# ZhenlongYuan/TSAR-MVS

Hardware: AMD Instinct MI355X
Metric: depthmap Mpixels/sec (ETH3D full-res, 8 iters) (higher is better)
Workload: dtype f32

## Files before the change

### tsar-mvs_amd/csrc/pm_core.h

```cpp
#pragma once
#include <type_traits>

#include "tsar_device_math.h"

#define PM_BLOCK 256
#define PM_RW 32

#include "pm_tap_common.h"

template <bool QUAD, bool DIFF = false>
DEVFN float sample_bilinear(const DevView& vw, int w, int h, int qpitch, float u, float v, bool q8 = false) {
    u = fminf(fmaxf(u, -1.0f), (float)w);
    v = fminf(fmaxf(v, -1.0f), (float)h);
    const float fu = floorf(u), fv = floorf(v);
    float ax = u - fu, ay = v - fv;
    if (q8) { ax = rintf(ax * 256.0f) * 0.00390625f; ay = rintf(ay * 256.0f) * 0.00390625f; }
    const int iu = (int)fu, iv = (int)fv;
    float t00, t10, t01, t11;
    if (QUAD) {
        const uint32_t off = (uint32_t)(__mul24(iv + 1, qpitch) + iu + 1) * 4u;
        const uint32_t q = *(global_u32_ptr)((const char __attribute__((address_space(1)))*)vw.quad + off);
        t00 = (float)(q & 0xffu);
        t10 = (float)((q >> 8) & 0xffu);
        t01 = (float)((q >> 16) & 0xffu);
// ... 130 lines not shown
DEVFN float add_prior_term(const DevScene* __restrict__ sc, int x, int y, const float4& n4, float D, float c) {
    const float4* pp = sc->prior;
    if (pp == nullptr) return c;
    typedef float prior_entry __attribute__((ext_vector_type(4)));
    const prior_entry q = ((const __attribute__((address_space(1))) prior_entry*)pp)[y * sc->w + x];
    const float Dp = q.w;
    const float a = fabsf(D - Dp);
    const float rel = a / Dp;
    const float dclip = sc->prior_depth_clip, nclip = sc->prior_normal_clip;
    const float r_d = rel < dclip ? rel / dclip : 1.0f;
    const float s = 1.0f - ((n4.x * q.x + n4.y * q.y) + n4.z * q.z);
    const float s0 = s < 0.0f ? 0.0f : s;
    const float r_n = s < nclip ? s0 / nclip : 1.0f;
    const float t = (sc->prior_weight_depth * r_d) + (sc->prior_weight_normal * r_n);
    return Dp > 0.0f ? c + t : c;
}

template <int NB, int HR, bool STRICT, bool QUAD, int V = 0, int BLK = PM_BLOCK>
DEVFN float multiview_cost(const DevScene* __restrict__ sc, const typename TileOf<QUAD>::type* tile, int tw, int own, const float* wts, const PixelRef& pr,
                           int x, int y, const float4& n4, int& beview, float& ratio, bool prune = false, float cost_now = 0.0f, int* skipped = nullptr) {
    constexpr bool GEOM = (V & TSAR_V_GEOM) != 0;
    constexpr bool PRUNE = (V & TSAR_V_PRUNE) != 0;
    static_assert(!PRUNE || !GEOM, "the bound speaks of the photometric cost alone");
    constexpr int VT = V & ~(TSAR_V_GEOM | TSAR_V_REDRAW | TSAR_V_PRUNE);
    float best[NB];
#pragma unroll
    for (int k = 0; k < NB; k++) best[k] = __builtin_inff();
    const int num = sc->n_sel;
    int valid = 0, bv = -1;
    float cmin = __builtin_inff();
    float depth_h = 0.0f;
    if constexpr (GEOM) depth_h = plane_depth(sc->ref, n4, x, y);
    int vi_next = sc->sel[0];
    for (int i = 0; i < num; i++) {
        const int vi = vi_next;
        vi_next = sc->sel[i + 1 < num ? i + 1 : i];
        float c;
        if constexpr ((VT & TSAR_V_LUT) != 0) c = view_cost_lut<STRICT, (VT >> 11) & 7, (VT & TSAR_V_BUF) != 0 && !STRICT, (VT & TSAR_V_MIX) != 0 && !STRICT>(sc, sc->view[vi], tile, tw, own, wts, pr, x, y, n4);
        else if constexpr (QUAD && HR == 5 && r5_production_variant(VT) && PRUNE) {
            static_assert((VT & 250) == 250 && !STRICT, "pruning instantiations exist for the fast row-wise loop");
            ViewPrune vp;
            vp.on = prune; vp.skipped = false;
            vp.cost_now = cmin < cost_now ? TSAR_MAXCOST : cost_now;
            c = view_cost_r5<false, true, true, (VT & TSAR_V_BUF) != 0, (VT & TSAR_V_MIX) != 0, BLK, 0, true>(sc, sc->view[vi], tile, tw, own, wts, pr, x, y, n4, &vp);
            if (vp.skipped) *skipped += 1;
        } else if constexpr (QUAD && HR == 5 && r5_production_variant(VT))
            c = view_cost_r5<STRICT, (VT & 128) != 0 && !STRICT, (VT & 8) != 0, (VT & TSAR_V_BUF) != 0, (VT & TSAR_V_MIX) != 0, BLK>(sc, sc->view[vi], tile, tw, own, wts, pr, x, y, n4);
#ifdef TSAR_EXPERIMENTS
        else if constexpr (QUAD && HR == 5 && r5_diag_variant(VT))
            c = view_cost_r5<false, true, true, true, true, BLK, (VT & 4194304) ? 1 : 2>(sc, sc->view[vi], tile, tw, own, wts, pr, x, y, n4);
#endif
        else {
            static_assert(VT == 0, "unknown tap-loop variant");
            c = view_cost_generic<HR, STRICT, QUAD, BLK>(sc, sc->view[vi], tile, tw, own, wts, pr, x, y, n4);
        }
        auto vmin = [](float a, float b) { float r; asm("v_min_f32 %0, %1, %2" : "=v"(r) : "v"(a), "v"(b)); return r; };
        auto vmax = [](float a, float b) { float r; asm("v_max_f32 %0, %1, %2" : "=v"(r) : "v"(a), "v"(b)); return r; };
        c = vmin(c, TSAR_MAXCOST);
        valid -= (int32_t)__float_as_uint(c - TSAR_MAXCOST) >> 31;
        if constexpr (GEOM) c = c + geom_term(sc, sc->view[vi], vi, x, y, depth_h);
        {
            const uint32_t worse = (uint32_t)((int32_t)__float_as_uint(cmin - c) >> 31);
            asm("v_bfi_b32 %0, %1, %2, %3" : "=v"(bv) : "v"(worse), "v"(bv), "s"(vi));
            cmin = vmin(cmin, c);
        }
        float v = c;
#pragma unroll
        for (int k = 0; k < NB; k++) {
            const float lo = vmin(best[k], v), hi = vmax(best[k], v);
            best[k] = lo;
            v = hi;
// ... 37 lines not shown
```

### tsar-mvs_amd/csrc/pm_init.hip

```cpp
#include "pm_init_impl.h"

template <bool INIT, bool REDRAW = false>
static int launch_full(tsar_ctx* ctx, const float4* planes, float* c, float4* n, int32_t* bv, float* rt) {
    if (every_pixel_takes_lut(ctx)) return launch_pm_full_lut(ctx, INIT, REDRAW, planes, c, n, bv, rt);
    return with_tap_config(ctx, [&](auto cfg) { return launch_full_g<decltype(cfg), INIT, REDRAW>(cfg, ctx, planes, c, n, bv, rt); });
}

int launch_pm_init(tsar_ctx* ctx) { return launch_full<true>(ctx, nullptr, ctx->buf[0].c, ctx->buf[0].n4, nullptr, nullptr); }
int launch_pm_cost_planes(tsar_ctx* ctx, const float4* planes, float* cost, int32_t* beview, float* ratio) {
    return launch_full<false>(ctx, planes, cost, nullptr, beview, ratio);
}
int launch_pm_rescore(tsar_ctx* ctx, const float4* planes, float* cost, float4* n, int32_t* beview, float* ratio) {
    return launch_full<true, true>(ctx, planes, cost, n, beview, ratio);
}
```

### tsar-mvs_amd/csrc/pm_init_impl.h

```cpp
#pragma once
#include "pm_dispatch.h"

#define FULL_RH 8

template <int NB, int HR, bool STRICT, bool QUAD, bool INIT, int V = 0>
__global__ __launch_bounds__(PM_BLOCK) void pm_full_kernel(const DevScene* __restrict__ sc, const float4* __restrict__ planes_in,
                                                           float* __restrict__ c_out, float4* __restrict__ n_out,
                                                           int32_t* __restrict__ beview_out, float* __restrict__ ratio_out, int tiles_x,
                                                           int n_tiles, int strip_w) {
    extern __shared__ __attribute__((aligned(16))) unsigned char lds_raw[];
    typedef typename TileOf<QUAD>::type TileT;
    const int hr = HR > 0 ? HR : sc->hrad, vr = HR > 0 ? HR : sc->vrad;
    const int tw = PM_RW + 2 * hr, th = FULL_RH + 2 * vr;
    constexpr bool LUTW = (V & TSAR_V_LUT) != 0;
    const size_t lut_bytes = LUTW ? (size_t)(sc->lut_classes + 1) * 1024 : 0;
    TileT* tile = (TileT*)(lds_raw + lut_bytes);
    float* wts = LUTW ? (float*)lds_raw : (float*)(lds_raw + tile_bytes<QUAD>(tw, th)) + threadIdx.x;
    if constexpr (LUTW) build_weight_lut<PM_BLOCK>(sc, wts);
    const int t = xcd_tile(blockIdx.x, n_tiles);
    int tix, tiy;
    strip_tile(t, tiles_x, n_tiles / tiles_x, strip_w, tix, tiy);
    const int ty0 = tiy * FULL_RH, tx0 = tix * PM_RW;
    stage_ref_tile<FULL_RH, TileT>(sc, tile, tx0, ty0, hr, vr, LUTW ? LUT_TILE_PAD_ROWS : 0);
    __syncthreads();
// ... 41 lines not shown
        n4 = planes_in[p];
    }
    if constexpr (REDRAW) n_out[p] = n4;
    PixelRef pr;
    if constexpr (LUTW) pr = hoist_reference_lut(sc, tile, tw, own, wts);
    else pr = hoist_reference<HR, TileT>(tile, tw, own, wts, hr, vr);
    float cost = TSAR_MAXCOST, rt = 0.f;
    int bv = -1;
    if (pr.textured) cost = multiview_cost<NB, HR, STRICT, QUAD, V>(sc, tile, tw, own, wts, pr, x, y, n4, bv, rt);
    c_out[p] = cost;
    if (!INIT || REDRAW) {
        if (beview_out) beview_out[p] = bv;
        if (ratio_out) ratio_out[p] = rt;
    }
}

template <int NB, int HR, bool STRICT, bool QUAD, bool INIT, int V = 0>
static int launch_full_t(tsar_ctx* ctx, const float4* planes, float* c, float4* n, int32_t* bv, float* rt) {
    auto kern = pm_full_kernel<NB, HR, STRICT, QUAD, INIT, V>;
    TapGrid g;
    if (const int rc = tap_grid(ctx, kern, FULL_RH, PM_BLOCK, QUAD, V, 0, g)) return rc;
    {
        ScopedKernelTimer tm(ctx, (INIT && (V & TSAR_V_REDRAW)) ? "pm_rescore" : INIT ? "pm_init" : "pm_cost_planes");
        hipLaunchKernelGGL(kern, dim3(g.n_tiles), dim3(PM_BLOCK), g.lds, ctx->stream, ctx->dscene, planes, c, n, bv, rt, g.tiles_x, g.n_tiles, strip_width(ctx->strip_w, g.tiles_x));
    }
    TSAR_HIP_TRY(ctx, hipGetLastError());
    return TSAR_OK;
}

template <class Cfg, bool INIT, bool REDRAW = false>
static int launch_full_g(Cfg, tsar_ctx* ctx, const float4* planes, float* c, float4* n, int32_t* bv, float* rt) {
    constexpr int NB = Cfg::NB, HR = Cfg::HR, V = Cfg::V;
    constexpr bool STRICT = Cfg::STRICT, QUAD = Cfg::QUAD;
    static_assert(INIT || !REDRAW, "only the initialising form redraws");
    if constexpr (REDRAW) return launch_full_t<NB, HR, STRICT, QUAD, true, V | TSAR_V_GEOM | TSAR_V_REDRAW>(ctx, planes, c, n, bv, rt);
    else if (scene_has_terms(ctx->hscene)) return launch_full_t<NB, HR, STRICT, QUAD, INIT, V | TSAR_V_GEOM>(ctx, planes, c, n, bv, rt);
    else return launch_full_t<NB, HR, STRICT, QUAD, INIT, V>(ctx, planes, c, n, bv, rt);
}
```

### tsar-mvs_amd/csrc/pm_sweep.hip

```cpp
#include "pm_sweep_impl.h"

__global__ void d16_probe_kernel(uint32_t* out) {
    __shared__ unsigned short t[64];
    t[threadIdx.x] = (unsigned short)(0x4300u + threadIdx.x);
    __syncthreads();
    uint32_t r = 0xffffffffu;
    const uint32_t addr = (uint32_t)(uintptr_t)(const __attribute__((address_space(3))) unsigned short*)(t + threadIdx.x);
    asm volatile("ds_read_u16_d16_hi %0, %1\n\ts_waitcnt lgkmcnt(0)" : "+v"(r) : "v"(addr));
    out[threadIdx.x] = r;
}
bool probe_d16_hi_zeroes(tsar_ctx* ctx) {
    CallFrame f(ctx, "d16 probe", nullptr, false);
    uint32_t h[64];
    uint32_t* d = f.out(h, 64, TSAR_MEM_HOST);
    if (f.ok()) {
        hipLaunchKernelGGL(d16_probe_kernel, dim3(1), dim3(64), 0, ctx->stream, d);
        f.launched();
    }
    bool ok = f.finish() == TSAR_OK;
    for (int i = 0; ok && i < 64; i++) ok = h[i] == ((0x4300u + i) << 16);
    return ok;
}

template <int NB, int HR>
static int launch_sweep_nh(tsar_ctx* ctx, int colour, const PlaneBuf& a, const PlaneBuf& b, const PlaneBuf& c, uint32_t sid, int dp, int dr) {
    const bool strict = ctx->hscene.flags & TSAR_FLAG_STRICT_DIV, quad = ctx->hscene.use_quad;
    const bool buf = ctx->buffer_gather && ctx->sweeps_done >= (strict ? (ctx->buffer_from > 2 ? ctx->buffer_from : 2) : ctx->buffer_from);
    const int v = ctx->variant;
    if constexpr ((NB == 2 || NB == 4) && HR == 5)
    if (quad && !(ctx->hscene.flags & TSAR_FLAG_TEX_FILTER_8BIT) && (v == 250 || v == 122 || (v == 114 && NB == 2))) {
#define SWEEP_R5(S, V, B) (buf ? launch_sweep_g<NB, 5, S, true, (V) | TSAR_V_BUF, B>(ctx, colour, a, b, c, sid, dp, dr) : launch_sweep_g<NB, 5, S, true, V, B>(ctx, colour, a, b, c, sid, dp, dr))
        const bool mix = buf && !strict && v == 250 && ctx->hscene.n_sel > 0 && ctx->hscene.view[ctx->hscene.sel[0]].dquad != nullptr;
#define SWEEP_R5_FAST250_ALL(B) (mix ? launch_sweep_g<NB, 5, false, true, 250 | TSAR_V_BUF | TSAR_V_MIX, B>(ctx, colour, a, b, c, sid, dp, dr) : SWEEP_R5(false, 250, B))
        const bool prune = NB == 2 && !strict && v == 250 && ctx->prune && ctx->prune_steps > 0 && dr && ctx->call_launch >= ctx->prune_from &&
                           ctx->hscene.cost_comb == TSAR_COMB_BEST_N && ctx->hscene.n_best == 1 && !scene_has_terms(ctx->hscene);
#define SWEEP_R5_PRUNE(B) (mix ? launch_sweep_t<2, 5, false, true, 250 | TSAR_V_BUF | TSAR_V_MIX | TSAR_V_PRUNE, B>(ctx, colour, a, b, c, sid, dp, dr) \
                           : buf ? launch_sweep_t<2, 5, false, true, 250 | TSAR_V_BUF | TSAR_V_PRUNE, B>(ctx, colour, a, b, c, sid, dp, dr)              \
                                 : launch_sweep_t<2, 5, false, true, 250 | TSAR_V_PRUNE, B>(ctx, colour, a, b, c, sid, dp, dr))
#define SWEEP_R5_FAST250(B) (prune ? SWEEP_R5_PRUNE(B) : SWEEP_R5_FAST250_ALL(B))
        if constexpr (NB == 2) {
            const int tiles256 = ((ctx->hscene.w + PM_RW - 1) / PM_RW) * ((ctx->hscene.h + 15) / 16);
            bool small = tiles256 < SWEEP_SMALL_IMAGE_TILES;
            if (ctx->force_block) small = ctx->force_block == 128;
            if (small && v != 114) {
                if (strict) return SWEEP_R5(true, 122, 128);
                return v == 250 ? SWEEP_R5_FAST250(128) : launch_sweep_g<2, 5, false, true, 122, 128>(ctx, colour, a, b, c, sid, dp, dr);
            }
            if (v == 114) return strict ? launch_sweep_g<2, 5, true, true, 114>(ctx, colour, a, b, c, sid, dp, dr) : launch_sweep_g<2, 5, false, true, 114>(ctx, colour, a, b, c, sid, dp, dr);
        }
        if (strict) return SWEEP_R5(true, 122, PM_BLOCK);
        return v == 250 ? SWEEP_R5_FAST250(PM_BLOCK) : launch_sweep_g<NB, 5, false, true, 122>(ctx, colour, a, b, c, sid, dp, dr);
#undef SWEEP_R5_FAST250
#undef SWEEP_R5_PRUNE
#undef SWEEP_R5_FAST250_ALL
#undef SWEEP_R5
    }
    constexpr int NBG = NB == 4 ? 32 : NB;
    if (strict) return quad ? launch_sweep_g<NBG, HR, true, true>(ctx, colour, a, b, c, sid, dp, dr) : launch_sweep_g<NBG, HR, true, false>(ctx, colour, a, b, c, sid, dp, dr);
    return quad ? launch_sweep_g<NBG, HR, false, true>(ctx, colour, a, b, c, sid, dp, dr) : launch_sweep_g<NBG, HR, false, false>(ctx, colour, a, b, c, sid, dp, dr);
}

int launch_pm_sweep(tsar_ctx* ctx, int colour, const PlaneBuf& same_in, const PlaneBuf& other, const PlaneBuf& same_out, uint32_t stream_id,
// ... 20 lines not shown
```

### tsar-mvs_amd/csrc/pm_sweep_experiments.hip

```cpp
#include "pm_sweep_impl.h"

int launch_pm_sweep_experiment(tsar_ctx* ctx, int colour, const PlaneBuf& a, const PlaneBuf& b, const PlaneBuf& c, uint32_t sid, int dp, int dr, int* launched) {
    *launched = 0;
    const DevScene& hs = ctx->hscene;
    const int need = views_in_cost(hs);
    const bool strict = hs.flags & TSAR_FLAG_STRICT_DIV;
    if (!(hs.use_quad && hs.hrad == 5 && hs.vrad == 5 && need <= 2) || (hs.flags & TSAR_FLAG_TEX_FILTER_8BIT)) return TSAR_OK;
#define EXP(S, V) case V: *launched = 1; return launch_sweep_t<2, 5, S, true, V>(ctx, colour, a, b, c, sid, dp, dr)
    int variant = getenv("TSAR_VARIANT_NOW") ? atoi(getenv("TSAR_VARIANT_NOW")) : ctx->variant;
    if ((variant & TSAR_V_MIX) && !(hs.n_sel > 0 && hs.view[hs.sel[0]].dquad != nullptr)) {
        ctx->err = "TSAR_VARIANT: the difference-texture tap loop needs the views' dquad textures (fast mode, TSAR_MIX_GATHER on)";
        return TSAR_ERR_STATE;
    }
    if (strict) return TSAR_OK;
    switch (variant) {
        EXP(false, 131322);
        EXP(false, 2228474);
        EXP(false, 6422778);
        EXP(false, 10617082);
        default: return TSAR_OK;
    }
#undef EXP
}
```

### tsar-mvs_amd/csrc/pm_sweep_impl.h

```cpp
#pragma once
#include "pm_dispatch.h"

#define SWEEP_SMALL_IMAGE_TILES 3072

#define CAND_SAME (1 << 30)

DEVFN void select_candidates(const DevScene* __restrict__ sc, const float* __restrict__ c_same, const float* __restrict__ c_other,
                             int x, int y, int cand[8]) {
    const int col = sc->w, row = sc->h;
    const int p = y * col + x;
    const bool fix_seed = sc->flags & TSAR_FLAG_FIX_DOWN_FAR_SEED, fix_cmp = sc->flags & TSAR_FLAG_FIX_RIGHT_FAR_CMP;
    float cmin;
    int cp, cs;
#pragma unroll
    for (int k = 0; k < 8; k++) cand[k] = -1;
    if (y > 2) {
        cp = p - 3 * col; cmin = c_other[cp];
#pragma unroll
        for (int i = 1; i < 11; ++i)
            if (y > 2 + 2 * i) { const int q = p - (3 + 2 * i) * col; const float v = c_other[q]; if (v < cmin) { cmin = v; cp = q; } }
        cand[0] = cp;
    }
    if (y < row - 3) {
        cp = p + 3 * col;
// ... 404 lines not shown
#else
    constexpr size_t lds_pad = 0;
#endif
    SweepMemo memo;
    memo.cand = ctx->memo_cand; memo.seq = ctx->memo_seq; memo.changed = ctx->changed_seq;
    memo.launch = ctx->launch_seq; memo.valid_from = ctx->memo_valid_from;
    memo.mode = (ctx->memo_mode && ctx->memo_cand && ctx->cost_consistent && !ctx->final_text) ? 1 : 0;
    memo.prune_steps = ((V & TSAR_V_PRUNE) != 0 && do_refine && ctx->call_launch >= ctx->prune_from) ? ctx->prune_steps : 0;
    memo.prune_counts = (V & TSAR_V_PRUNE) != 0 ? ctx->prune_counts : nullptr;
    bool packed = false;
    if constexpr (sweep_has_packed_form<HR, QUAD, V>())
        packed = memo.mode && do_prop && ctx->compact_from >= 0 && ctx->call_launch >= ctx->compact_from;
    auto kern = pm_sweep_kernel<NB, HR, STRICT, QUAD, V, BLK, false>;
    if constexpr (sweep_has_packed_form<HR, QUAD, V>())
        if (packed) kern = pm_sweep_kernel<NB, HR, STRICT, QUAD, V, BLK, true>;
    const size_t slots = packed ? 6 * (size_t)BLK : 0;
    TapGrid g;
    if (const int rc = tap_grid(ctx, kern, SWEEP_RH, BLK, QUAD, V, lds_pad + slots, g)) return rc;
    memo.slot_off = packed ? (int)(g.lds - slots) : 0;
    {
        ScopedKernelTimer tm(ctx, (V & TSAR_V_GEOM) ? "pm_sweep_geom" : "pm_sweep");
        ScopedKernelTimer tm_packed(ctx, packed ? "pm_sweep_packed" : nullptr);
        ScopedKernelTimer tm_prune(ctx, (V & TSAR_V_PRUNE) ? "pm_sweep_prune" : nullptr);
        hipLaunchKernelGGL(kern, dim3(g.n_tiles), dim3(BLK), g.lds, ctx->stream, ctx->dscene, colour, same_in.c, same_in.n4, other.c,
                           other.n4, same_out.c, same_out.n4, ctx->ratio, ctx->beview, stream_id, do_prop, do_refine, g.tiles_x, g.n_tiles,
                           ctx->cost_consistent ? 1 : 0, strip_width(ctx->strip_w, g.tiles_x), ctx->final_text, memo);
    }
    TSAR_HIP_TRY(ctx, hipGetLastError());
    return TSAR_OK;
}

template <int NB, int HR, bool STRICT, bool QUAD, int V = 0, int BLK = PM_BLOCK>
static int launch_sweep_g(tsar_ctx* ctx, int colour, const PlaneBuf& same_in, const PlaneBuf& other, const PlaneBuf& same_out,
                          uint32_t stream_id, int do_prop, int do_refine) {
    if (scene_has_terms(ctx->hscene)) return launch_sweep_t<NB, HR, STRICT, QUAD, V | TSAR_V_GEOM, BLK>(ctx, colour, same_in, other, same_out, stream_id, do_prop, do_refine);
    return launch_sweep_t<NB, HR, STRICT, QUAD, V, BLK>(ctx, colour, same_in, other, same_out, stream_id, do_prop, do_refine);
}
```

### tsar-mvs_amd/csrc/pm_tap_common.h

```cpp
#pragma once

typedef const uint32_t __attribute__((address_space(1)))* global_u32_ptr;
typedef const float __attribute__((address_space(1)))* global_f32_ptr;

template <bool STRICT, bool ROW = false>
DEVFN void tap_line_base(const float* H, float a, float& bx, float& by, float& bz) {
    bx = STRICT ? H[0] * a : fma_(H[ROW ? 1 : 0], a, H[2]);
    by = STRICT ? H[3] * a : fma_(H[ROW ? 4 : 3], a, H[5]);
    bz = STRICT ? H[6] * a : fma_(H[ROW ? 7 : 6], a, H[8]);
}
template <bool STRICT, bool ROW = false>
DEVFN void tap_homogeneous(const float* H, float t, float bx, float by, float bz, float& X, float& Y, float& Z) {
    X = fma_(H[ROW ? 0 : 1], t, bx); Y = fma_(H[ROW ? 3 : 4], t, by); Z = fma_(H[ROW ? 6 : 7], t, bz);
    if (STRICT) { X += H[2]; Y += H[5]; Z += H[8]; }
}
DEVFN void pixel_homogeneous(const float* H, float xi, float yj, float& X, float& Y, float& Z) {
    float bx, by, bz;
    tap_line_base<false>(H, xi, bx, by, bz);
    tap_homogeneous<false>(H, yj, bx, by, bz, X, Y, Z);
}

template <bool STRICT, bool GUARD>
DEVFN void tap_divide(float X, float Y, float Z, float& u, float& v) {
    if (STRICT) {
// ... 35 lines not shown
DEVFN void pin_quad_base(uint64_t base, uint32_t& lo, uint32_t& hi) {
    lo = __builtin_amdgcn_readfirstlane((uint32_t)base);
    hi = __builtin_amdgcn_readfirstlane((uint32_t)(base >> 32));
    asm volatile("" : "+s"(lo), "+s"(hi));
}
typedef uint32_t u32x4s __attribute__((ext_vector_type(4)));
template <bool MIX>
DEVFN u32x4s quad_descriptor(uint64_t base, int rows, int qp) {
    u32x4s rsrc;
    rsrc.x = __builtin_amdgcn_readfirstlane((uint32_t)base);
    rsrc.y = __builtin_amdgcn_readfirstlane(((uint32_t)(base >> 32) & 0xffffu) | ((MIX ? 8u : 4u) << 16));
    rsrc.z = __builtin_amdgcn_readfirstlane((uint32_t)(qp * rows - 1));
    rsrc.w = 0x00020000u;
    asm volatile("" : "+s"(rsrc));
    return rsrc;
}

template <bool MIX>
DEVFN std::conditional_t<MIX, uint64_t, uint32_t> buffer_gather(int lin, u32x4s rsrc) {
    std::conditional_t<MIX, uint64_t, uint32_t> q;
    if constexpr (MIX) asm volatile("buffer_load_dwordx2 %0, %1, %2, 0 idxen" : "=v"(q) : "v"(lin), "s"(rsrc));
    else asm volatile("buffer_load_dword %0, %1, %2, 0 idxen" : "=v"(q) : "v"(lin), "s"(rsrc));
    return q;
}
template <bool FAST>
DEVFN float blend_texels(float t00, float t10, float t01, float t11, float ax, float ay) {
    if (FAST) {
        const float d1 = t10 - t00, d2 = t01 - t00, d3 = (t11 - t01) - d1;
        return fma_(ay, fma_(ax, d3, d2), fma_(ax, d1, t00));
    }
    const float top = fma_(ax, t10 - t00, t00);
    const float bot = fma_(ax, t11 - t01, t01);
    return fma_(ay, bot - top, top);
}
template <bool FAST>
DEVFN float blend_quad(uint32_t q, float ax, float ay) {
    float t00, t10, t01, t11;
    asm("v_cvt_f32_ubyte0 %0, %1" : "=v"(t00) : "v"(q));
    asm("v_cvt_f32_ubyte1 %0, %1" : "=v"(t10) : "v"(q));
    asm("v_cvt_f32_ubyte2 %0, %1" : "=v"(t01) : "v"(q));
    asm("v_cvt_f32_ubyte3 %0, %1" : "=v"(t11) : "v"(q));
    return blend_texels<FAST>(t00, t10, t01, t11, ax, ay);
}
DEVFN float blend_dquad(uint64_t q2, float ax, float ay) {
    const uint32_t lo = (uint32_t)q2, hi = (uint32_t)(q2 >> 32);
    float ta, tb;
// ... 68 lines not shown
```

### tsar-mvs_amd/csrc/pm_tap_r5.h

```cpp
#pragma once

#define PM_PRUNE_FIRST_LINE 2
#define PM_PRUNE_LAST_LINE 4

template <bool STRICT, bool ROW, bool D16, bool BUF, bool MIX, int BLK, int DIAG = 0, bool PRUNE = false>
DEVFN float view_cost_r5(const DevScene* __restrict__ sc, const DevView& vw, const unsigned short* tile, int tw, int own, const float* wts,
                         const PixelRef& pr, int x, int y, const float4& n4, ViewPrune* vp = nullptr) {
    static_assert(!(STRICT && ROW), "the row-wise walk changes the summation order: fast mode only");
    static_assert(!PRUNE || (ROW && D16 && !STRICT && DIAG == 0), "the partial-window bound is written for the fast row-wise loop");
    static_assert(!MIX || (BUF && !STRICT), "the half-float difference texture serves the fast arithmetic's blend through buffer loads");
    const int w = sc->w, h = sc->h, qp = sc->quad_pitch;
    const int qorg = quad_border_bytes(qp);
    float H[9];
    if (STRICT) plane_homography(sc->ref, vw, n4, H, sc->k_sparse != 0);
    else plane_homography_fast(sc->ref, vw, n4, H);
    float sum_src = 0.f, sum_src_src = 0.f, sum_ref_src = 0.f;
    bool need_clamp;
    if (!STRICT) {
        float Xc, Yc, Zc;
        pixel_homogeneous(H, (float)x, (float)y, Xc, Yc, Zc);
        const float a = fabsf(H[0]) + fabsf(H[1]), b = fabsf(H[3]) + fabsf(H[4]), c = fabsf(H[6]) + fabsf(H[7]);
        const float Zmin = fma_(-5.0f, c, Zc);
        const float r = __builtin_amdgcn_rcpf(Zmin * Zc);
        const float r5 = 5.0f * r, rc = Zmin * r;
        const float du = fma_(a, Zc, fabsf(Xc) * c) * r5, dv = fma_(b, Zc, fabsf(Yc) * c) * r5;
        const float uc = Xc * rc, vc = Yc * rc;
        const bool inside = Zmin > 0.0f && fminf(uc - du, vc - dv) >= 1.5f && uc + du <= (float)(w - 1) - 1.5f && vc + dv <= (float)(h - 1) - 1.5f;
        need_clamp = !__all(inside);
    } else {
        bool inside = true;
        float zmin = __builtin_inff(), zmax = 0.0f;
#pragma unroll
        for (int c = 0; c < 4; c++) {
// ... 22 lines not shown
        static_assert(!UNR || (ROW && D16), "the unrolled form is written for the row-wise walk with D16 window loads");
        const float xi = (float)((ROW ? y : x) + i);
        float bx, by, bz;
        tap_line_base<STRICT, ROW>(H, xi, bx, by, bz);
        const int line = (i + 5) >> 1;
        float rcol[6];
        f32x2 wcol[3];
        {
            constexpr int U = BLK / 64, S = ROW ? 6 : 1;
            const uint32_t wa = (uint32_t)(uintptr_t)(const __attribute__((address_space(3))) float*)(wts + (UNR ? 0 : (ROW ? line : 6 * line) * BLK));
#pragma unroll
            for (int k = 0; k < 3; k++)
                asm("ds_read2st64_b32 %0, %1 offset0:%2 offset1:%3" : "=v"(wcol[k]) : "v"(wa), "n"(2 * U * S * k + (UNR ? U * line : 0)), "n"(2 * U * S * k + U * S + (UNR ? U * line : 0)), "v"(bz));
        }
        if (D16) {
            const uint32_t a0 = (uint32_t)(uintptr_t)(const __attribute__((address_space(3))) unsigned short*)(UNR ? tile + own - 5 * tw - 5 : ROW ? tile + own + i * tw - 5 : tile + own + i - 5 * tw);
#pragma unroll
            for (int jj = 0; jj < 6; jj++)
                asm("ds_read_u16_d16_hi %0, %1 offset:%2" : "=v"(rcol[jj]) : "v"(a0), "n"((ROW ? jj * 4 : jj * 2 * (PM_RW + 10) * 2) + (UNR ? line * 2 * (PM_RW + 10) * 2 : 0)), "v"(bz));
        }
        float ax[6], ay[6];
        uint32_t q[6];
        uint64_t q2[6];
        __builtin_amdgcn_s_setprio(3);
#pragma unroll
        for (int jj = 0; jj < 6; jj++) {
            const float yj = (float)((ROW ? x : y) + 2 * jj - 5);
            float X, Y, Z;
            tap_homogeneous<STRICT, ROW>(H, yj, bx, by, bz, X, Y, Z);
            const float uhi = (float)(w - 1), vhi = (float)(h - 1);
            int lin;
            tap_position<STRICT, CLAMP>(X, Y, Z, uhi, vhi, qp, ax[jj], ay[jj], lin);
            if (MIX && DIAG == 1) {
                q2[jj] = ((uint64_t)(uint32_t)~lin << 32) | (uint32_t)lin;
            } else if (MIX && DIAG == 2) {
                uint32_t la;
                asm("v_bfe_u32 %0, %1, 0, 12" : "=v"(la) : "v"(lin));
                asm volatile("ds_read_b64 %0, %1" : "=v"(q2[jj]) : "v"(la << 3));
            } else if (MIX) {
                q2[jj] = buffer_gather<true>(lin, rsrc);
            } else if (BUF) {
                q[jj] = buffer_gather<false>(lin, rsrc);
            } else {
                const uint32_t off2 = (uint32_t)lin << 2;
                q[jj] = *(global_u32_ptr)((const char __attribute__((address_space(1)))*)(uintptr_t)(((uint64_t)qb_hi << 32) | qb_lo) + off2);
            }
        }
        __builtin_amdgcn_sched_barrier(0);
        __builtin_amdgcn_s_setprio(0);
        __builtin_amdgcn_sched_barrier(0);
#pragma unroll
        for (int jj = 0; jj < 6; jj++) {
            if (MIX && DIAG == 1) {
            } else if (MIX && DIAG == 2) {
                if (jj == 0) asm("s_waitcnt lgkmcnt(5)" : "+v"(q2[0]), "+v"(rcol[0]), "+v"(rcol[1]), "+v"(rcol[2]), "+v"(rcol[3]), "+v"(rcol[4]), "+v"(rcol[5]),
                                 "+v"(wcol[0]), "+v"(wcol[1]), "+v"(wcol[2]) : "v"(q2[5]));
                else asm("s_waitcnt lgkmcnt(%2)" : "+v"(q2[jj]), "+v"(sum_src_src) : "n"(5 - jj), "v"(q2[5]));
            } else if (MIX) {
                if (jj == 0) asm("s_waitcnt vmcnt(5)" : "+v"(q2[0]) : "v"(q2[5]));
                if (jj == 1) asm("s_waitcnt vmcnt(4)" : "+v"(q2[1]), "+v"(sum_src_src) : "v"(q2[5]));
                if (jj == 2) asm("s_waitcnt vmcnt(3)" : "+v"(q2[2]), "+v"(sum_src_src) : "v"(q2[5]));
                if (jj == 3) asm("s_waitcnt vmcnt(2)" : "+v"(q2[3]), "+v"(sum_src_src) : "v"(q2[5]));
                if (jj == 4) asm("s_waitcnt vmcnt(1)" : "+v"(q2[4]), "+v"(sum_src_src) : "v"(q2[5]));
                if (jj == 5) asm("s_waitcnt vmcnt(0)" : "+v"(q2[5]), "+v"(sum_src_src));
            } else if (BUF) {
                if (jj == 0) asm("s_waitcnt vmcnt(5)" : "+v"(q[0]) : "v"(q[5]));
                if (jj == 1) asm("s_waitcnt vmcnt(4)" : "+v"(q[1]), "+v"(sum_src_src) : "v"(q[5]));
                if (jj == 2) asm("s_waitcnt vmcnt(3)" : "+v"(q[2]), "+v"(sum_src_src) : "v"(q[5]));
                if (jj == 3) asm("s_waitcnt vmcnt(2)" : "+v"(q[3]), "+v"(sum_src_src) : "v"(q[5]));
                if (jj == 4) asm("s_waitcnt vmcnt(1)" : "+v"(q[4]), "+v"(sum_src_src) : "v"(q[5]));
                if (jj == 5) asm("s_waitcnt vmcnt(0)" : "+v"(q[5]), "+v"(sum_src_src));
            }
            float s;
            if (MIX) s = blend_dquad(q2[jj], ax[jj], ay[jj]);
            else s = blend_quad<!STRICT>(q[jj], ax[jj], ay[jj]);
            if (jj == 0 && DIAG != 2) {
                if (D16)
                    asm("s_waitcnt lgkmcnt(0)" : "+v"(rcol[0]), "+v"(rcol[1]), "+v"(rcol[2]), "+v"(rcol[3]), "+v"(rcol[4]), "+v"(rcol[5]),
                        "+v"(wcol[0]), "+v"(wcol[1]), "+v"(wcol[2]), "+v"(s));
                else
                    asm("s_waitcnt lgkmcnt(0)" : "+v"(wcol[0]), "+v"(wcol[1]), "+v"(wcol[2]), "+v"(s));
            }
            const float r = D16 ? rcol[jj] : tile_value(ROW ? tile[own + i * tw + (2 * jj - 5)] : tile[own + (2 * jj - 5) * tw + i]);
            const float wt = wcol[jj >> 1][jj & 1];
            const TapSums t = tap_accumulate<STRICT>(TapSums{sum_src, sum_src_src, sum_ref_src}, wt, r, s);
            sum_src = t.src; sum_src_src = t.src_src; sum_ref_src = t.ref_src;
        }
    };
    auto pruned = [&](int line) {
        if constexpr (PRUNE) {
            if (vp->on && line >= PM_PRUNE_FIRST_LINE - 1 && line < PM_PRUNE_LAST_LINE) {
                float pa_w = 0.f, pa_r = 0.f, pa_rr = 0.f;
#pragma unroll 1
                for (int l = 0; l <= line; l++) {
// ... 30 lines not shown
```

### tsar-mvs_amd/csrc/tsar_api.hip

```cpp
#include <math.h>
#include <stdio.h>
#include <stdlib.h>
#include <string.h>

#include <algorithm>

#include "tsar_dev.h"

ScopedKernelTimer::ScopedKernelTimer(tsar_ctx* c, const char* name) : ctx(c) {
    if (!ctx->timing || !name) return;
    for (size_t k = 0; k < ctx->timers.size(); k++)
        if (ctx->timers[k].name == name) ti = (int)k;
    if (ti < 0) {
        ctx->timers.emplace_back();
        ctx->timers.back().name = name;
        ti = (int)ctx->timers.size() - 1;
    }
    if (hipEventCreate(&e0) != hipSuccess) { ti = -1; return; }
    if (hipEventCreate(&e1) != hipSuccess) { hipEventDestroy(e0); ti = -1; return; }
    hipEventRecord(e0, ctx->stream);
}
ScopedKernelTimer::~ScopedKernelTimer() {
    if (ti < 0) return;
    hipEventRecord(e1, ctx->stream);
// ... 157 lines not shown

extern "C" const char* tsar_version(void) {
#ifdef TSAR_EXPERIMENTS
    return "tsar-mvs_amd 0.2.0 (gfx950) +experiments";
#else
    return "tsar-mvs_amd 0.2.0 (gfx950)";
#endif
}

static void read_knobs(tsar_ctx* ctx) {
    auto num = [](const char* name, int dflt) { const char* e = getenv(name); return e && e[0] ? atoi(e) : dflt; };
    auto on = [](const char* name, bool dflt) { const char* e = getenv(name); return e && e[0] ? e[0] != '0' : dflt; };
    ctx->variant = num("TSAR_VARIANT", ctx->variant);
    ctx->buffer_gather = on("TSAR_BUFFER_GATHER", true);
    ctx->mix_gather = on("TSAR_MIX_GATHER", true);
    ctx->strip_w = num("TSAR_STRIP", -1);
    ctx->buffer_from = num("TSAR_BUFFER_FROM", 1);
    ctx->force_block = num("TSAR_BLOCK", 0);
    ctx->memo_mode = num("TSAR_MEMO", 1);
    ctx->compact_from = num("TSAR_COMPACT_FROM", 6);
    ctx->prune = num("TSAR_PRUNE", 1);
    ctx->prune_steps = std::min(std::max(num("TSAR_PRUNE_STEPS", 2), 0), 8);
    ctx->prune_from = num("TSAR_PRUNE_FROM", 1);
    ctx->lut_mode = num("TSAR_LUT", 1);
    ctx->ransac_wgs = num("TSAR_RANSAC_WGS", 8);
    ctx->ransac_chain = num("TSAR_RANSAC_CHAIN", 8);
    ctx->ransac_lookahead = num("TSAR_RANSAC_LOOKAHEAD", 0);
    ctx->ransac_poll_limit = num("TSAR_RANSAC_POLL_LIMIT", 1 << 15);
    ctx->ransac_cooperative = on("TSAR_RANSAC_COOPERATIVE", true);
    ctx->ransac_force_fallback = on("TSAR_RANSAC_FORCE_FALLBACK", false);
    ctx->trace_host = getenv("TSAR_TRACE_HOST") != nullptr;
#ifdef TSAR_EXPERIMENTS
    ctx->lds_pad = (size_t)num("TSAR_LDS_PAD", 0);
#endif
}

extern "C" int tsar_create(int device, tsar_ctx** out) {
    if (!out) return TSAR_ERR_INVALID;
    *out = nullptr;
    int n = 0;
    if (hipGetDeviceCount(&n) != hipSuccess || n <= 0) return TSAR_ERR_HIP;
    if (device < 0 || device >= n) return TSAR_ERR_INVALID;
    if (hipSetDevice(device) != hipSuccess) return TSAR_ERR_HIP;
    tsar_ctx* ctx = new (std::nothrow) tsar_ctx();
    if (!ctx) return TSAR_ERR_NOMEM;
    ctx->device = device;
// ... 1062 lines not shown
```

### tsar-mvs_amd/csrc/tsar_dev.h

```cpp
#pragma once
#include <hip/hip_runtime.h>
#include <stdint.h>
#include <stdio.h>
#include <stdlib.h>

#include <chrono>
#include <string>
#include <vector>

#include "../../include/tsar.h"

#define TSAR_LUT_LINES 32
#define TSAR_LUT_TAPS 40
#define TSAR_LUT_MAX_CLASSES 144
#define TSAR_MAX_SELECTED 32

struct DevView {
    float K[9];
    float R[9];
    float t[3];
    float t_abs_lo;
    float A[9];
    float b[3];
    float t_abs_hi;
// ... 28 lines not shown
    DevRef ref;
    int sel[TSAR_MAX_VIEWS];
    DevView view[TSAR_MAX_VIEWS];
    int lut_classes;
    int lut_row_major;
    int lut_chunk;
    int lut_pad_taps;
    int lut_d2[TSAR_LUT_MAX_CLASSES];
    uint32_t tap_row[TSAR_LUT_LINES * TSAR_LUT_TAPS + 8];
    const float* geom_depth[TSAR_MAX_VIEWS];
    float geom_back[TSAR_MAX_VIEWS][12];
    float geom_weight, geom_clip, geom_clip_sq;
    int geom_on;
    const float4* prior;
    float prior_weight_depth, prior_weight_normal, prior_depth_clip, prior_normal_clip;
};
static inline bool scene_has_terms(const DevScene& s) { return s.geom_on != 0 || s.prior != nullptr; }

#define TSAR_V_LUT 1024
#define TSAR_V_BUF 131072
#define TSAR_V_MIX 2097152
#define TSAR_V_GEOM 16777216
#define TSAR_V_PRUNE 67108864
#define TSAR_V_REDRAW 33554432

struct PlaneBuf {
    float* c;
    float4* n4;
};

struct KernelTimer {
    std::string name;
    int launches = 0;
    float total_ms = 0.f;
    std::vector<std::pair<hipEvent_t, hipEvent_t>> pending;
};

struct ScratchArena {
    char* base = nullptr;
    size_t cap = 0;
    size_t wanted = 0;
};

struct tsar_ctx {
    int device = 0;
    hipStream_t stream = nullptr;
// ... 9 lines not shown
    PlaneBuf buf[2]{};
    float *ratio = nullptr, *depth = nullptr, *scale = nullptr, *lrdiff = nullptr, *confid = nullptr, *fakedepth = nullptr;
    int32_t *beview = nullptr, *canny = nullptr;
    float4* out4 = nullptr;
    bool have_out = false;
    bool cost_consistent = false;
    int n_regions = 0;
    float *region_text = nullptr, *region_size = nullptr;
    float4* region_n4 = nullptr;
    int exact_sqrt_probe = 0;
    int exact_div_probe = 0;
    int sweeps_done = 0;
    int32_t* memo_cand = nullptr;
    uint32_t* memo_seq = nullptr;
    uint32_t* changed_seq = nullptr;
    uint32_t launch_seq = 0;
    uint32_t memo_valid_from = 1;
    int call_launch = 0;
    int memo_mode = 1;
    int compact_from = 6;
    int prune = 1;
    int prune_steps = 2;
    int prune_from = 1;
    uint32_t* prune_counts = nullptr;
    std::vector<tsar_camera> cams;
    bool views_u8 = false;
    float4* resize4 = nullptr;
    bool have_resize = false;
    const float* final_text = nullptr;
    std::vector<float*> geom_maps;
    float4* prior = nullptr;
    int variant = 2;
    bool mix_gather = true;
    bool buffer_gather = true;
    int strip_w = -1;
    int buffer_from = 1;
    int force_block = 0;
    int lut_mode = 1;
    int ransac_wgs = 8;
    int ransac_chain = 8;
    int ransac_lookahead = 0;
    int ransac_poll_limit = 1 << 15;
    bool ransac_cooperative = true;
    bool ransac_force_fallback = false;
    bool trace_host = false;
#ifdef TSAR_EXPERIMENTS
// ... 164 lines not shown
    } while (0)

static inline int install_regions(tsar_ctx* ctx, int n) {
    ctx->n_regions = 0;
    TRY(dev_alloc(ctx, &ctx->region_text, (size_t)n));
    TRY(dev_alloc(ctx, &ctx->region_size, (size_t)n));
    TRY(dev_alloc(ctx, &ctx->region_n4, (size_t)n));
    TSAR_HIP_TRY(ctx, hipMemsetAsync(ctx->region_n4, 0, (size_t)n * 16, ctx->stream));
    return TSAR_OK;
}

struct ScopedKernelTimer {
    tsar_ctx* ctx;
    int ti = -1;
    hipEvent_t e0 = nullptr, e1 = nullptr;
    ScopedKernelTimer(tsar_ctx* c, const char* name);
    ~ScopedKernelTimer();
};

int launch_build_quad(tsar_ctx* ctx, const float* img, uint32_t* quad, int w, int h, int* nonintegral_flag);
int launch_expand_u8(tsar_ctx* ctx, const uint8_t* in, float* out, size_t n);
int launch_build_dquad(tsar_ctx* ctx, const uint32_t* quad, uint2* dquad, int w, int h);
int launch_pm_init(tsar_ctx* ctx);
bool probe_d16_hi_zeroes(tsar_ctx* ctx);
int launch_pm_sweep(tsar_ctx* ctx, int colour, const PlaneBuf& same_in, const PlaneBuf& other, const PlaneBuf& same_out,
                    uint32_t stream_id, int do_prop, int do_refine);
int launch_pm_sweep_lut(tsar_ctx* ctx, int colour, const PlaneBuf& same_in, const PlaneBuf& other, const PlaneBuf& same_out, uint32_t stream_id,
                        int do_prop, int do_refine);
int launch_pm_full_lut(tsar_ctx* ctx, bool init, bool redraw, const float4* planes, float* c, float4* n, int32_t* bv, float* rt);
int lut_chunk_taps(int taps_per_line);
static inline bool lut_path_forced(const tsar_ctx* ctx) { return ctx->lut_mode == 2; }
static inline bool lut_path_applies(const tsar_ctx* ctx) {
    const bool off = ctx->lut_mode == 0;
    const DevScene& hs = ctx->hscene;
    const bool d16_ok = (hs.flags & TSAR_FLAG_STRICT_DIV) || (ctx->variant & 8);
    return !off && d16_ok && hs.use_quad && hs.lut_classes > 0;
}
int launch_pm_sweep_experiment(tsar_ctx* ctx, int colour, const PlaneBuf& same_in, const PlaneBuf& other, const PlaneBuf& same_out, uint32_t stream_id,
                               int do_prop, int do_refine, int* launched);
int launch_pm_cost_planes(tsar_ctx* ctx, const float4* planes, float* cost, int32_t* beview, float* ratio);
int launch_pm_rescore(tsar_ctx* ctx, const float4* planes, float* cost, float4* n, int32_t* beview, float* ratio);
int launch_pm_upsample(tsar_ctx* ctx, const float4* coarse, int cw, int ch);
int launch_pm_upsample_merge(tsar_ctx* ctx, const float4* coarse, int cw, int ch);
int launch_pm_upsample_lut(tsar_ctx* ctx, bool merge, const float4* coarse, int cw, int ch);
int launch_pyr_down(tsar_ctx* ctx, const float* src, int w, int h, void* dst, bool u8);
int launch_geom_pyramid(tsar_ctx* ctx, const float* src, int w, int h, float* dst);
// ... 24 lines not shown
```

Before: 47.55.

## Pair adjacent tap gathers into one 16-byte load with byte-permute extraction

Adds a paired-gather variant of the box-11 row-wise tap loop. Each even tap issues a 16-byte global load, and the following odd tap takes its texel via v_perm from that vector when its index lies within 3 dwords. Otherwise it falls back to a separate 4-byte load. The variant is enabled by default for init and sweep when the scene has no extra terms and the buffer/prune paths are off. It aims to cut the number of gather instructions at the cost of wider loads, extra permute ALU work and a divergent fallback load.

```diff
diff --git a/tsar-mvs_amd/csrc/pm_core.h b/tsar-mvs_amd/csrc/pm_core.h
--- a/tsar-mvs_amd/csrc/pm_core.h
+++ b/tsar-mvs_amd/csrc/pm_core.h
@@ -176,7 +176,9 @@
     constexpr bool GEOM = (V & TSAR_V_GEOM) != 0;
     constexpr bool PRUNE = (V & TSAR_V_PRUNE) != 0;
     static_assert(!PRUNE || !GEOM, "the bound speaks of the photometric cost alone");
-    constexpr int VT = V & ~(TSAR_V_GEOM | TSAR_V_REDRAW | TSAR_V_PRUNE);
+    constexpr bool PAIR = (V & TSAR_V_PAIR) != 0;
+    static_assert(!PAIR || (!PRUNE && !GEOM), "the paired gathers exist for the plain fast box-11 kernels");
+    constexpr int VT = V & ~(TSAR_V_GEOM | TSAR_V_REDRAW | TSAR_V_PRUNE | TSAR_V_PAIR);
     float best[NB];
 #pragma unroll
     for (int k = 0; k < NB; k++) best[k] = __builtin_inff();
@@ -198,9 +200,14 @@
             vp.cost_now = cmin < cost_now ? TSAR_MAXCOST : cost_now;
             c = view_cost_r5<false, true, true, (VT & TSAR_V_BUF) != 0, (VT & TSAR_V_MIX) != 0, BLK, 0, true>(sc, sc->view[vi], tile, tw, own, wts, pr, x, y, n4, &vp);
             if (vp.skipped) *skipped += 1;
+        } else if constexpr (QUAD && HR == 5 && PAIR && VT == 250) {
+            static_assert(!STRICT, "the paired gathers exist for the fast row-wise loop");
+            c = view_cost_r5<false, true, true, false, false, BLK, 0, false, true>(sc, sc->view[vi], tile, tw, own, wts, pr, x, y, n4);
         } else if constexpr (QUAD && HR == 5 && r5_production_variant(VT))
             c = view_cost_r5<STRICT, (VT & 128) != 0 && !STRICT, (VT & 8) != 0, (VT & TSAR_V_BUF) != 0, (VT & TSAR_V_MIX) != 0, BLK>(sc, sc->view[vi], tile, tw, own, wts, pr, x, y, n4);
 #ifdef TSAR_EXPERIMENTS
+        else if constexpr (QUAD && HR == 5 && PAIR && VT == (250 | 4194304))
+            c = view_cost_r5<false, true, true, false, false, BLK, 3, false, true>(sc, sc->view[vi], tile, tw, own, wts, pr, x, y, n4);
         else if constexpr (QUAD && HR == 5 && r5_diag_variant(VT))
             c = view_cost_r5<false, true, true, true, true, BLK, (VT & 4194304) ? 1 : 2>(sc, sc->view[vi], tile, tw, own, wts, pr, x, y, n4);
 #endif
diff --git a/tsar-mvs_amd/csrc/pm_init.hip b/tsar-mvs_amd/csrc/pm_init.hip
--- a/tsar-mvs_amd/csrc/pm_init.hip
+++ b/tsar-mvs_amd/csrc/pm_init.hip
@@ -6,7 +6,17 @@
     return with_tap_config(ctx, [&](auto cfg) { return launch_full_g<decltype(cfg), INIT, REDRAW>(cfg, ctx, planes, c, n, bv, rt); });
 }
 
-int launch_pm_init(tsar_ctx* ctx) { return launch_full<true>(ctx, nullptr, ctx->buf[0].c, ctx->buf[0].n4, nullptr, nullptr); }
+int launch_pm_init(tsar_ctx* ctx) {
+    float* const c = ctx->buf[0].c;
+    float4* const n = ctx->buf[0].n4;
+    if (every_pixel_takes_lut(ctx)) return launch_pm_full_lut(ctx, true, false, nullptr, c, n, nullptr, nullptr);
+    return with_tap_config(ctx, [&](auto cfg) {
+        typedef decltype(cfg) Cfg;
+        if constexpr (Cfg::NB == 2 && Cfg::HR == 5 && !Cfg::STRICT && Cfg::QUAD && Cfg::V == 250)
+            if ((ctx->pair & 1) && !scene_has_terms(ctx->hscene)) return launch_pm_init_pair(ctx);
+        return launch_full_g<Cfg, true, false>(cfg, ctx, nullptr, c, n, nullptr, nullptr);
+    });
+}
 int launch_pm_cost_planes(tsar_ctx* ctx, const float4* planes, float* cost, int32_t* beview, float* ratio) {
     return launch_full<false>(ctx, planes, cost, nullptr, beview, ratio);
 }
diff --git a/tsar-mvs_amd/csrc/pm_init_impl.h b/tsar-mvs_amd/csrc/pm_init_impl.h
--- a/tsar-mvs_amd/csrc/pm_init_impl.h
+++ b/tsar-mvs_amd/csrc/pm_init_impl.h
@@ -87,6 +87,7 @@
     if (const int rc = tap_grid(ctx, kern, FULL_RH, PM_BLOCK, QUAD, V, 0, g)) return rc;
     {
         ScopedKernelTimer tm(ctx, (INIT && (V & TSAR_V_REDRAW)) ? "pm_rescore" : INIT ? "pm_init" : "pm_cost_planes");
+        ScopedKernelTimer tm_pair(ctx, (V & TSAR_V_PAIR) ? "pm_init_pair" : nullptr);
         hipLaunchKernelGGL(kern, dim3(g.n_tiles), dim3(PM_BLOCK), g.lds, ctx->stream, ctx->dscene, planes, c, n, bv, rt, g.tiles_x, g.n_tiles, strip_width(ctx->strip_w, g.tiles_x));
     }
     TSAR_HIP_TRY(ctx, hipGetLastError());
diff --git a/tsar-mvs_amd/csrc/pm_pair.hip b/tsar-mvs_amd/csrc/pm_pair.hip
--- /dev/null
+++ b/tsar-mvs_amd/csrc/pm_pair.hip
@@ -0,0 +1,12 @@
+#include "pm_init_impl.h"
+#include "pm_sweep_impl.h"
+
+int launch_pm_init_pair(tsar_ctx* ctx) {
+    return launch_full_t<2, 5, false, true, true, 250 | TSAR_V_PAIR>(ctx, nullptr, ctx->buf[0].c, ctx->buf[0].n4, nullptr, nullptr);
+}
+
+int launch_pm_sweep_pair(tsar_ctx* ctx, int block, int colour, const PlaneBuf& same_in, const PlaneBuf& other, const PlaneBuf& same_out,
+                         uint32_t stream_id, int do_prop, int do_refine) {
+    if (block == 128) return launch_sweep_t<2, 5, false, true, 250 | TSAR_V_PAIR, 128>(ctx, colour, same_in, other, same_out, stream_id, do_prop, do_refine);
+    return launch_sweep_t<2, 5, false, true, 250 | TSAR_V_PAIR, PM_BLOCK>(ctx, colour, same_in, other, same_out, stream_id, do_prop, do_refine);
+}
diff --git a/tsar-mvs_amd/csrc/pm_sweep.hip b/tsar-mvs_amd/csrc/pm_sweep.hip
--- a/tsar-mvs_amd/csrc/pm_sweep.hip
+++ b/tsar-mvs_amd/csrc/pm_sweep.hip
@@ -37,7 +37,8 @@
 #define SWEEP_R5_PRUNE(B) (mix ? launch_sweep_t<2, 5, false, true, 250 | TSAR_V_BUF | TSAR_V_MIX | TSAR_V_PRUNE, B>(ctx, colour, a, b, c, sid, dp, dr) \
                            : buf ? launch_sweep_t<2, 5, false, true, 250 | TSAR_V_BUF | TSAR_V_PRUNE, B>(ctx, colour, a, b, c, sid, dp, dr)              \
                                  : launch_sweep_t<2, 5, false, true, 250 | TSAR_V_PRUNE, B>(ctx, colour, a, b, c, sid, dp, dr))
-#define SWEEP_R5_FAST250(B) (prune ? SWEEP_R5_PRUNE(B) : SWEEP_R5_FAST250_ALL(B))
+        const bool pair = NB == 2 && !strict && v == 250 && !buf && !prune && (ctx->pair & 2) && !scene_has_terms(ctx->hscene);
+#define SWEEP_R5_FAST250(B) (prune ? SWEEP_R5_PRUNE(B) : pair ? launch_pm_sweep_pair(ctx, B, colour, a, b, c, sid, dp, dr) : SWEEP_R5_FAST250_ALL(B))
         if constexpr (NB == 2) {
             const int tiles256 = ((ctx->hscene.w + PM_RW - 1) / PM_RW) * ((ctx->hscene.h + 15) / 16);
             bool small = tiles256 < SWEEP_SMALL_IMAGE_TILES;
diff --git a/tsar-mvs_amd/csrc/pm_sweep_experiments.hip b/tsar-mvs_amd/csrc/pm_sweep_experiments.hip
--- a/tsar-mvs_amd/csrc/pm_sweep_experiments.hip
+++ b/tsar-mvs_amd/csrc/pm_sweep_experiments.hip
@@ -18,6 +18,7 @@
         EXP(false, 2228474);
         EXP(false, 6422778);
         EXP(false, 10617082);
+        EXP(false, 138412282);
         default: return TSAR_OK;
     }
 #undef EXP
diff --git a/tsar-mvs_amd/csrc/pm_sweep_impl.h b/tsar-mvs_amd/csrc/pm_sweep_impl.h
--- a/tsar-mvs_amd/csrc/pm_sweep_impl.h
+++ b/tsar-mvs_amd/csrc/pm_sweep_impl.h
@@ -450,6 +450,7 @@
         ScopedKernelTimer tm(ctx, (V & TSAR_V_GEOM) ? "pm_sweep_geom" : "pm_sweep");
         ScopedKernelTimer tm_packed(ctx, packed ? "pm_sweep_packed" : nullptr);
         ScopedKernelTimer tm_prune(ctx, (V & TSAR_V_PRUNE) ? "pm_sweep_prune" : nullptr);
+        ScopedKernelTimer tm_pair(ctx, (V & TSAR_V_PAIR) ? "pm_sweep_pair" : nullptr);
         hipLaunchKernelGGL(kern, dim3(g.n_tiles), dim3(BLK), g.lds, ctx->stream, ctx->dscene, colour, same_in.c, same_in.n4, other.c,
                            other.n4, same_out.c, same_out.n4, ctx->ratio, ctx->beview, stream_id, do_prop, do_refine, g.tiles_x, g.n_tiles,
                            ctx->cost_consistent ? 1 : 0, strip_width(ctx->strip_w, g.tiles_x), ctx->final_text, memo);
diff --git a/tsar-mvs_amd/csrc/pm_tap_common.h b/tsar-mvs_amd/csrc/pm_tap_common.h
--- a/tsar-mvs_amd/csrc/pm_tap_common.h
+++ b/tsar-mvs_amd/csrc/pm_tap_common.h
@@ -81,6 +81,14 @@
     if constexpr (MIX) asm volatile("buffer_load_dwordx2 %0, %1, %2, 0 idxen" : "=v"(q) : "v"(lin), "s"(rsrc));
     else asm volatile("buffer_load_dword %0, %1, %2, 0 idxen" : "=v"(q) : "v"(lin), "s"(rsrc));
     return q;
+}
+typedef u32x4s u32x4s_a4 __attribute__((aligned(4)));
+typedef const u32x4s_a4 __attribute__((address_space(1)))* global_u32x4_a4_ptr;
+DEVFN uint32_t pick_dword(u32x4s a, uint32_t k) {
+    const uint32_t b0 = (uint32_t)((int32_t)(k << 31) >> 31), b1 = (uint32_t)((int32_t)(k << 30) >> 31);
+    const uint32_t s0 = (b0 & 0x04040404u) | 0x03020100u, s1 = (b1 & 0x04040404u) | 0x03020100u;
+    const uint32_t lo = __builtin_amdgcn_perm(a.y, a.x, s0), hi = __builtin_amdgcn_perm(a.w, a.z, s0);
+    return __builtin_amdgcn_perm(hi, lo, s1);
 }
 template <bool FAST>
 DEVFN float blend_texels(float t00, float t10, float t01, float t11, float ax, float ay) {
diff --git a/tsar-mvs_amd/csrc/pm_tap_r5.h b/tsar-mvs_amd/csrc/pm_tap_r5.h
--- a/tsar-mvs_amd/csrc/pm_tap_r5.h
+++ b/tsar-mvs_amd/csrc/pm_tap_r5.h
@@ -3,12 +3,14 @@
 #define PM_PRUNE_FIRST_LINE 2
 #define PM_PRUNE_LAST_LINE 4
 
-template <bool STRICT, bool ROW, bool D16, bool BUF, bool MIX, int BLK, int DIAG = 0, bool PRUNE = false>
+template <bool STRICT, bool ROW, bool D16, bool BUF, bool MIX, int BLK, int DIAG = 0, bool PRUNE = false, bool PAIR = false>
 DEVFN float view_cost_r5(const DevScene* __restrict__ sc, const DevView& vw, const unsigned short* tile, int tw, int own, const float* wts,
                          const PixelRef& pr, int x, int y, const float4& n4, ViewPrune* vp = nullptr) {
     static_assert(!(STRICT && ROW), "the row-wise walk changes the summation order: fast mode only");
     static_assert(!PRUNE || (ROW && D16 && !STRICT && DIAG == 0), "the partial-window bound is written for the fast row-wise loop");
     static_assert(!MIX || (BUF && !STRICT), "the half-float difference texture serves the fast arithmetic's blend through buffer loads");
+    static_assert(!PAIR || (ROW && D16 && !STRICT && !BUF && !MIX && !PRUNE), "the paired gathers are written for the plain fast row-wise loop on the byte texture");
+    static_assert(DIAG != 3 || PAIR, "DIAG 3 is a form of the paired loop");
     const int w = sc->w, h = sc->h, qp = sc->quad_pitch;
     const int qorg = quad_border_bytes(qp);
     float H[9];
@@ -77,6 +79,8 @@
         float ax[6], ay[6];
         uint32_t q[6];
         uint64_t q2[6];
+        int linv[6];
+        u32x4s wide[3];
         __builtin_amdgcn_s_setprio(3);
 #pragma unroll
         for (int jj = 0; jj < 6; jj++) {
@@ -96,10 +100,19 @@
                 q2[jj] = buffer_gather<true>(lin, rsrc);
             } else if (BUF) {
                 q[jj] = buffer_gather<false>(lin, rsrc);
+            } else if constexpr (PAIR) {
+                linv[jj] = lin;
+                if ((jj & 1) == 0) wide[jj >> 1] = *(global_u32x4_a4_ptr)((const char __attribute__((address_space(1)))*)(uintptr_t)(((uint64_t)qb_hi << 32) | qb_lo) + ((uint32_t)lin << 2));
             } else {
                 const uint32_t off2 = (uint32_t)lin << 2;
                 q[jj] = *(global_u32_ptr)((const char __attribute__((address_space(1)))*)(uintptr_t)(((uint64_t)qb_hi << 32) | qb_lo) + off2);
             }
+        }
+        if constexpr (PAIR && DIAG != 3) {
+#pragma unroll
+            for (int jj = 1; jj < 6; jj += 2)
+                if ((uint32_t)(linv[jj] - linv[jj - 1]) > 3u)
+                    q[jj] = *(global_u32_ptr)((const char __attribute__((address_space(1)))*)(uintptr_t)(((uint64_t)qb_hi << 32) | qb_lo) + ((uint32_t)linv[jj] << 2));
         }
         __builtin_amdgcn_sched_barrier(0);
         __builtin_amdgcn_s_setprio(0);
@@ -125,6 +138,13 @@
                 if (jj == 3) asm("s_waitcnt vmcnt(2)" : "+v"(q[3]), "+v"(sum_src_src) : "v"(q[5]));
                 if (jj == 4) asm("s_waitcnt vmcnt(1)" : "+v"(q[4]), "+v"(sum_src_src) : "v"(q[5]));
                 if (jj == 5) asm("s_waitcnt vmcnt(0)" : "+v"(q[5]), "+v"(sum_src_src));
+            }
+            if constexpr (PAIR) {
+                if ((jj & 1) == 0) q[jj] = wide[jj >> 1].x;
+                else {
+                    const uint32_t k = (uint32_t)(linv[jj] - linv[jj - 1]);
+                    if (DIAG == 3 || k <= 3u) q[jj] = pick_dword(wide[jj >> 1], k);
+                }
             }
             float s;
             if (MIX) s = blend_dquad(q2[jj], ax[jj], ay[jj]);
diff --git a/tsar-mvs_amd/csrc/tsar_api.hip b/tsar-mvs_amd/csrc/tsar_api.hip
--- a/tsar-mvs_amd/csrc/tsar_api.hip
+++ b/tsar-mvs_amd/csrc/tsar_api.hip
@@ -203,6 +203,7 @@
     ctx->prune = num("TSAR_PRUNE", 1);
     ctx->prune_steps = std::min(std::max(num("TSAR_PRUNE_STEPS", 2), 0), 8);
     ctx->prune_from = num("TSAR_PRUNE_FROM", 1);
+    ctx->pair = num("TSAR_PAIR", 3);
     ctx->lut_mode = num("TSAR_LUT", 1);
     ctx->ransac_wgs = num("TSAR_RANSAC_WGS", 8);
     ctx->ransac_chain = num("TSAR_RANSAC_CHAIN", 8);
diff --git a/tsar-mvs_amd/csrc/tsar_dev.h b/tsar-mvs_amd/csrc/tsar_dev.h
--- a/tsar-mvs_amd/csrc/tsar_dev.h
+++ b/tsar-mvs_amd/csrc/tsar_dev.h
@@ -74,6 +74,7 @@
 #define TSAR_V_MIX 2097152
 #define TSAR_V_GEOM 16777216
 #define TSAR_V_PRUNE 67108864
+#define TSAR_V_PAIR 134217728
 #define TSAR_V_REDRAW 33554432
 
 struct PlaneBuf {
@@ -129,6 +130,7 @@
     int prune = 1;
     int prune_steps = 2;
     int prune_from = 1;
+    int pair = 3;
     uint32_t* prune_counts = nullptr;
     std::vector<tsar_camera> cams;
     bool views_u8 = false;
@@ -339,6 +341,9 @@
 int launch_expand_u8(tsar_ctx* ctx, const uint8_t* in, float* out, size_t n);
 int launch_build_dquad(tsar_ctx* ctx, const uint32_t* quad, uint2* dquad, int w, int h);
 int launch_pm_init(tsar_ctx* ctx);
+int launch_pm_init_pair(tsar_ctx* ctx);
+int launch_pm_sweep_pair(tsar_ctx* ctx, int block, int colour, const PlaneBuf& same_in, const PlaneBuf& other, const PlaneBuf& same_out,
+                         uint32_t stream_id, int do_prop, int do_refine);
 bool probe_d16_hi_zeroes(tsar_ctx* ctx);
 int launch_pm_sweep(tsar_ctx* ctx, int colour, const PlaneBuf& same_in, const PlaneBuf& other, const PlaneBuf& same_out,
                     uint32_t stream_id, int do_prop, int do_refine);
```

After: 48.55, median of 6. +2.1%, better.
